# thuanz123/enhancing-transformers

Measured on AMD Instinct MI355X. Metric: images/sec ViT-VQGAN-base 256px stage-1 train; VQ argmin match-rate, higher is better.
Workload: dtype fp16; 1 GPU; imagenet_vitvq_base.yaml AE training step (1 fwd + 1 bwd + grad all-reduce + AdamW), loss = 1.0*L2 + 1.0*codebook (LPIPS/GAN weights 0), K=8192 x 32 l2-normalised codes, fp32 master weights, fp16 MFMA operands / fp32 accumulate, dynamic loss scale (now 65536; device-side inf/nan step skip + GradScaler update rule); per_gpu_batch=128, global_batch=128, image=256x256, parallelism=dp1, hip_graph_replay=False

## Files before the change

enhancing-transformers_amd/csrc/attention_kernels.h:

```cpp
#ifndef ATT_TAIL
#error "attention_kernels.h is included with ATT_TAIL (0 | 1) and ATT_K (the kernel names) defined"
#endif
#include "attention_tile_loop.h"

template <typename OT>
__device__ __forceinline__ void ATT_K(fwd, exact)(const uint16_t* __restrict__ qkv, int B, int N, int H, float scale_log2, uint16_t* __restrict__ out,
                                               float* __restrict__ lse, unsigned char (*smem)[2][ATT_TILE_BYTES], int blk, int head) {
  const int t = threadIdx.x, lane = t & 63, wave = t >> 6;
  const int l31 = lane & 31, hi = lane >> 5;
  const int b = head / H, h = head - b * H;
  const int q0 = blk * 128 + wave * 32;
  const int64_t RS = (int64_t)3 * H * ATT_D;
  const uint16_t* Qp = qkv + (int64_t)b * N * RS + h * ATT_D;
  const uint16_t* Kp = Qp + H * ATT_D;
  const uint16_t* Vp = Kp + H * ATT_D;

  const bool active = ATT_SEL(q0 + l31 < N, q0 < N);
  const int qrow = ATT_SEL(min(q0 + l31, N - 1), active ? q0 + l31 : l31);
  s16x8 qf[4];
#pragma unroll
  for (int ds = 0; ds < 4; ++ds) qf[ds] = *reinterpret_cast<const s16x8*>(Qp + (int64_t)qrow * RS + ds * 16 + hi * 8);

  f32x16 o[2];
#pragma unroll
  for (int db = 0; db < 2; ++db)
#pragma unroll
    for (int r = 0; r < 16; ++r) o[db][r] = 0.f;
  float m_run = -__builtin_inff(), l_part = 0.f;

  const int nt = N / 64;
  u32x4 rk[2], rv[2];
#if ATT_TAIL
  if (nt == 0) {
    att_gload_clamped(rk, Kp, RS, 0, N, t);
    att_gload_clamped(rv, Vp, RS, 0, N, t);
  } else
#endif
  {
  att_gload(rk, Kp, RS, 0, t);
  att_gload(rv, Vp, RS, 0, t);
  }
  att_sstore(rk, smem[0][0], t);
  att_sstore(rv, smem[0][1], t);
#pragma unroll
  for (int ds = 0; ds < 4; ++ds) att_pin(qf[ds]);
  ATT_LOOP_ENTRY();
  __syncthreads();
  ATT_TILES_BEGIN(kt, nt)
    const int st = kt & 1;
#if ATT_TAIL
    if constexpr (LAST) {
    } else if (kt + 1 == nt) {
      att_gload_clamped(rk, Kp, RS, (kt + 1) * 64, N, t);
      att_gload_clamped(rv, Vp, RS, (kt + 1) * 64, N, t);
    } else
#else
    if (kt + 1 < nt)
#endif
    {
      att_gload(rk, Kp, RS, (kt + 1) * 64, t);
      att_gload(rv, Vp, RS, (kt + 1) * 64, t);
    }
    const unsigned char* kt_ = smem[st][0];
    const unsigned char* vt_ = smem[st][1];
    f32x16 s[2];
#pragma unroll
    for (int kb = 0; kb < 2; ++kb) {
#pragma unroll
      for (int r = 0; r < 16; ++r) s[kb][r] = ATT_SEL(LAST ? att_key_bias(kb, r, hi, N & 63) : 0.f, 0.f);
#pragma unroll
      for (int ds = 0; ds < 4; ++ds) s[kb] = MFMA32(att_frag_row(kt_, kb * 32, ds, l31, hi), qf[ds], s[kb]);
    }
    float mx = max3(s[0][0], s[0][1], s[0][2]);
#pragma unroll
    for (int r = 3; r < 15; r += 2) mx = max3(mx, s[0][r], s[0][r + 1]);
    mx = max3(mx, s[0][15], s[1][0]);
#pragma unroll
    for (int r = 1; r < 15; r += 2) mx = max3(mx, s[1][r], s[1][r + 1]);
    mx = xhalf_max(__builtin_fmaxf(mx, s[1][15]));
    const float mt = mx * scale_log2;
    if (kt == 0 || __builtin_amdgcn_ballot_w64(mt - m_run > 8.0f) != 0) {
      const float m_new = fmaxf(m_run, mt);
      const float alpha = __builtin_amdgcn_exp2f(m_run - m_new);
      m_run = m_new;
      l_part *= alpha;
#pragma unroll
      for (int db = 0; db < 2; ++db)
#pragma unroll
        for (int r = 0; r < 16; ++r) o[db][r] *= alpha;
    }
    float p[2][16];
    float psum = 0.f;
#pragma unroll
    for (int kb = 0; kb < 2; ++kb)
#pragma unroll
      for (int r = 0; r < 16; ++r) {
        p[kb][r] = __builtin_amdgcn_exp2f(s[kb][r] * scale_log2 - m_run);
        psum += p[kb][r];
      }
    l_part += psum;
#pragma unroll
    for (int kb = 0; kb < 2; ++kb)
#pragma unroll
      for (int c2 = 0; c2 < 2; ++c2) {
        const s16x8 pb = pack8<OT>(&p[kb][c2 * 8]);
#pragma unroll
        for (int db = 0; db < 2; ++db) o[db] = MFMA32(att_frag_tr(vt_, kb * 32 + 16 * c2, db, lane), pb, o[db]);
      }
    ATT_UNLESS_LAST {
    if (ATT_SEL(true, kt + 1 < nt)) {
      att_sstore(rk, smem[st ^ 1][0], t);
      att_sstore(rv, smem[st ^ 1][1], t);
    }
    __syncthreads();
    }
  ATT_TILES_END(kt, nt)
  const float l = l_part + __shfl_xor(l_part, 32, 64);
  const float inv = 1.0f / l;
  if (!active) return;
  uint16_t* op = out + ((int64_t)b * N + q0 + l31) * (H * ATT_D) + h * ATT_D;
#pragma unroll
  for (int db = 0; db < 2; ++db)
#pragma unroll
    for (int g4 = 0; g4 < 4; ++g4) {
      const int d0 = db * 32 + 8 * g4 + 4 * hi;
      u32x2 w = {pack2<OT>(o[db][g4 * 4 + 0] * inv, o[db][g4 * 4 + 1] * inv), pack2<OT>(o[db][g4 * 4 + 2] * inv, o[db][g4 * 4 + 3] * inv)};
      *reinterpret_cast<u32x2*>(op + d0) = w;
    }
  if (hi == 0) lse[((int64_t)b * H + h) * N + q0 + l31] = (m_run + __builtin_amdgcn_logf(l)) * 0.6931471805599453f;
}

#define ATT_PF 1
__host__ __device__ constexpr bool att_run_start(int k, int P, bool WHOLE) { return k == 0 || (!WHOLE && (k % P == 0 || k % P == 8)); }
__host__ __device__ constexpr int att_run_end(int I, int NF, int P, bool WHOLE) {
  int e = I + 1;
  while (e < NF && !att_run_start(e, P, WHOLE)) ++e;
  return e;
}
__host__ __device__ constexpr int att_pending(int I, int NF, int P, bool WHOLE) {
  int n = 0;
  for (int k = I + 1; k <= I + ATT_PF && k < att_run_end(I, NF, P, WHOLE); ++k) n += (k % P < 8) ? 1 : 2;
  return n;
}
template <int I, int NF, int P, bool WHOLE, typename REQ>
__device__ __forceinline__ void att_stream_request(REQ& req) {
  constexpr int E = att_run_end(I, NF, P, WHOLE);
  if constexpr (att_run_start(I, P, WHOLE)) att_static_for<I, (I + ATT_PF < E ? I + ATT_PF : E)>(req);
  if constexpr (I + ATT_PF < E) req(std::integral_constant<int, I + ATT_PF>{});
}

template <typename OT>
__global__ __launch_bounds__(256, 2) void ATT_K(fwd, kernel)(const uint16_t* __restrict__ qkv, int B, int N, int H, float scale_log2,
                                                          uint16_t* __restrict__ out, float* __restrict__ lse) {
  __shared__ __attribute__((aligned(16))) unsigned char smem[2][2][ATT_TILE_BYTES];
  int blk, head;
  if (!att_block_coords((N + 127) / 128, B * H, blk, head)) return;
  ATT_K(fwd, exact)<OT>(qkv, B, N, H, scale_log2, out, lse, smem, blk, head);
}

__device__ __forceinline__ float dot2_ones(uint32_t pk, float acc) {
  return __builtin_amdgcn_fdot2_f32_bf16(__builtin_bit_cast(bf16x2_t, pk), __builtin_bit_cast(bf16x2_t, 0x3f803f80u), acc, false);
}
template <typename OT>
__global__ __launch_bounds__(256, 2) void ATT_K(fwd, pre_kernel)(const uint16_t* __restrict__ qkv, int B, int N, int H, uint16_t* __restrict__ out, float* __restrict__ lse) {
  __shared__ __attribute__((aligned(16))) unsigned char smem[2][2][ATT_TILE_BYTES];
  int blk, head;
  if (!att_block_coords((N + 127) / 128, B * H, blk, head)) return;
  const int t = threadIdx.x, lane = t & 63, wave = t >> 6;
  const int l31 = lane & 31, hi = lane >> 5;
  const int b = head / H, h = head - b * H;
  const int q0 = blk * 128 + wave * 32;
  const int64_t RS = (int64_t)3 * H * ATT_D;
  const uint16_t* Qp = qkv + (int64_t)b * N * RS + h * ATT_D;
  const uint16_t* Kp = Qp + H * ATT_D;
  const uint16_t* Vp = Kp + H * ATT_D;
  const bool active = ATT_SEL(q0 + l31 < N, q0 < N);
  const int qrow = ATT_SEL(min(q0 + l31, N - 1), active ? q0 + l31 : l31);
  s16x8 qf[4];
#pragma unroll
  for (int ds = 0; ds < 4; ++ds) qf[ds] = *reinterpret_cast<const s16x8*>(Qp + (int64_t)qrow * RS + ds * 16 + hi * 8);
  f32x16 o[2], negm;
#pragma unroll
  for (int r = 0; r < 16; ++r) { o[0][r] = 0.f; o[1][r] = 0.f; negm[r] = 0.f; }
  float m_ref = 0.f;
  f32x2 l2[2] = {{0.f, 0.f}, {0.f, 0.f}};

  const int nt = N / 64;
  const int wave_u = __builtin_amdgcn_readfirstlane(wave);
  const unsigned ko0 = att_dma_lane_off((int)RS, lane, 0), ko1 = att_dma_lane_off((int)RS, lane, 1);
#if ATT_TAIL
  if (nt == 0) {
    att_dma_tile_clamped(Kp, RS, 0, N, smem[0][0], wave_u, lane);
    att_dma_tile_clamped(Vp, RS, 0, N, smem[0][1], wave_u, lane);
  } else
#endif
  {
  att_dma_tile(Kp, RS, 0, smem[0][0], wave_u, ko0, ko1);
  att_dma_tile(Vp, RS, 0, smem[0][1], wave_u, ko0, ko1);
  }
  unsigned ra[4], ta[2][2];
  att_ring_addresses(ra, ta, &smem[0][0][0], lane);
#pragma unroll
  for (int ds = 0; ds < 4; ++ds) att_pin(qf[ds]);
  ATT_LOOP_ENTRY();
  __syncthreads();
  ATT_TILES_BEGIN(kt, nt)
    const int st = kt & 1;
#if ATT_TAIL
    if constexpr (LAST) {
    } else if (kt + 1 == nt) {
      att_dma_tile_clamped(Kp, RS, (kt + 1) * 64, N, smem[st ^ 1][0], wave_u, lane);
      att_dma_tile_clamped(Vp, RS, (kt + 1) * 64, N, smem[st ^ 1][1], wave_u, lane);
    } else
#else
    if (kt + 1 < nt)
#endif
    {
      att_dma_tile(Kp, RS, (kt + 1) * 64, smem[st ^ 1][0], wave_u, ko0, ko1);
      att_dma_tile(Vp, RS, (kt + 1) * 64, smem[st ^ 1][1], wave_u, ko0, ko1);
    }
    constexpr int NF = 16;
    u32x4 fr[ATT_PF + 1];
    att_u64 tl[ATT_PF + 1], th[ATT_PF + 1];
    auto req = [&](auto ic) {
      constexpr int I = decltype(ic)::value, B = I % (ATT_PF + 1);
      if constexpr (I < 8) att_req_row<(I >> 2) * 32 * 128>(fr[B], ra[I & 3]);
      else att_req_tr<ATT_TILE_BYTES + (((I - 8) >> 2) * 32 + 16 * (((I - 8) >> 1) & 1)) * 128>(tl[B], th[B], ta[I & 1][0], ta[I & 1][1]);
    };
    f32x16 s[2];
    att_static_for<0, 8>([&](auto ic) {
      constexpr int I = decltype(ic)::value, kb = I >> 2, ds = I & 3, B = I % (ATT_PF + 1);
      att_stream_request<I, NF, 16, false>(req);
#if ATT_TAIL
      if constexpr (LAST && ds == 0) {
#pragma unroll
        for (int r = 0; r < 16; ++r) s[kb][r] = negm[r] + att_key_bias(kb, r, hi, N & 63);
      }
#endif
      s[kb] = MFMA32(att_take_row<att_pending(I, NF, 16, false)>(fr[B]), qf[ds], ATT_SEL(ds == 0 && !LAST, ds == 0) ? negm : s[kb]);
    });
    float mq[4];
#pragma unroll
    for (int c = 0; c < 4; ++c) {
      const f32x16& sv = s[c >> 1];
      const int r0 = (c & 1) * 8;
      mq[c] = max3(sv[r0], sv[r0 + 1], sv[r0 + 2]);
      mq[c] = max3(mq[c], sv[r0 + 3], sv[r0 + 4]);
      mq[c] = max3(mq[c], sv[r0 + 5], sv[r0 + 6]);
    }
    float mx = max3(mq[0], mq[1], s[0][7]);
    mx = max3(mx, mq[2], s[0][15]);
    mx = max3(mx, mq[3], s[1][7]);
    mx = xhalf_max(__builtin_fmaxf(mx, s[1][15]));
    if (kt == 0 || __builtin_amdgcn_ballot_w64(mx > 8.0f) != 0) {
      const float delta = kt == 0 ? mx : __builtin_fmaxf(mx, 0.f);
      if (kt != 0) {
        const float alpha = __builtin_amdgcn_exp2f(-delta);
        l2[0] *= alpha; l2[1] *= alpha;
#pragma unroll
        for (int db = 0; db < 2; ++db)
#pragma unroll
          for (int r = 0; r < 16; ++r) o[db][r] *= alpha;
      }
      m_ref += delta;
#pragma unroll
      for (int r = 0; r < 16; ++r) { s[0][r] -= delta; s[1][r] -= delta; negm[r] = -m_ref; }
    }
    s16x8 pb;
    att_static_for<8, 16>([&](auto ic) {
      constexpr int I = decltype(ic)::value, kb = (I - 8) >> 2, c2 = ((I - 8) >> 1) & 1, db = I & 1, B = I % (ATT_PF + 1);
      att_stream_request<I, NF, 16, false>(req);
      if constexpr (db == 0) {
        float p8[8];
#pragma unroll
        for (int j = 0; j < 8; ++j) p8[j] = __builtin_amdgcn_exp2f(s[kb][c2 * 8 + j]);
        const u32x4 pk = {pack2<OT>(p8[0], p8[1]), pack2<OT>(p8[2], p8[3]), pack2<OT>(p8[4], p8[5]), pack2<OT>(p8[6], p8[7])};
#pragma unroll
        for (int j = 0; j < 4; ++j) l2[j & 1] += (f32x2){p8[2 * j], p8[2 * j + 1]};
        pb = __builtin_bit_cast(s16x8, pk);
      }
      o[db] = MFMA32(att_take_tr<att_pending(I, NF, 16, false)>(tl[B], th[B]), pb, o[db]);
    });
    ATT_UNLESS_LAST {
    att_ring_advance(ra, ta, st);
    ATT_FENCE();
    __builtin_amdgcn_s_waitcnt(0x0F70);
    __syncthreads();
    }
  ATT_TILES_END(kt, nt)
  const float l_part = (l2[0][0] + l2[1][0]) + (l2[0][1] + l2[1][1]);
  const float l = l_part + __shfl_xor(l_part, 32, 64);
  const float inv = 1.0f / l;
  if (!active) return;
  uint16_t* op = out + ((int64_t)b * N + q0 + l31) * (H * ATT_D) + h * ATT_D;
#pragma unroll
  for (int db = 0; db < 2; ++db)
#pragma unroll
    for (int g4 = 0; g4 < 4; ++g4) {
      const int d0 = db * 32 + 8 * g4 + 4 * hi;
      u32x2 w = {pack2<OT>(o[db][g4 * 4 + 0] * inv, o[db][g4 * 4 + 1] * inv), pack2<OT>(o[db][g4 * 4 + 2] * inv, o[db][g4 * 4 + 3] * inv)};
      *reinterpret_cast<u32x2*>(op + d0) = w;
    }
  if (hi == 0) lse[((int64_t)b * H + h) * N + q0 + l31] = (m_ref + __builtin_amdgcn_logf(l)) * 0.6931471805599453f;
}

template <int MODE, typename OT>
__global__ __launch_bounds__(256, 3) void ATT_K(bwd, dq_kernel)(const uint16_t* __restrict__ qkv, const uint16_t* __restrict__ o, const uint16_t* __restrict__ d_o,
                                                             const float* __restrict__ lse, float* __restrict__ delta, int B, int N,
                                                             int H, float scale, float scale_log2, uint16_t* __restrict__ dqkv) {
  __shared__ __attribute__((aligned(16))) unsigned char smem[2][2][ATT_TILE_BYTES];
  const int t = threadIdx.x, lane = t & 63, wave = t >> 6;
  const int l31 = lane & 31, hi = lane >> 5;
  int blk, head;
  if (!att_block_coords((N + 127) / 128, B * H, blk, head)) return;
  const int b = head / H, h = head - b * H;
  const int q0 = blk * 128 + wave * 32;
  const int64_t RS = (int64_t)3 * H * ATT_D;
  const uint16_t* Qp = qkv + (int64_t)b * N * RS + h * ATT_D;
  const uint16_t* Kp = Qp + H * ATT_D;
  const uint16_t* Vp = Kp + H * ATT_D;
  const uint16_t* dOp = d_o + (int64_t)b * N * (H * ATT_D) + h * ATT_D;

  const bool active = ATT_SEL(q0 + l31 < N, q0 < N);
  const int qrow = ATT_SEL(min(q0 + l31, N - 1), active ? q0 + l31 : l31);
  s16x8 qf[4], dof[4];
#pragma unroll
  for (int ds = 0; ds < 4; ++ds) {
    qf[ds] = *reinterpret_cast<const s16x8*>(Qp + (int64_t)qrow * RS + ds * 16 + hi * 8);
    dof[ds] = *reinterpret_cast<const s16x8*>(dOp + (int64_t)qrow * (H * ATT_D) + ds * 16 + hi * 8);
  }
  const float lse_q = lse[((int64_t)b * H + h) * N + qrow] * 1.4426950408889634f;
  float dpart = 0.f;
#pragma unroll
  for (int ds = 0; ds < 4; ++ds) {
    const s16x8 of = *reinterpret_cast<const s16x8*>(o + ((int64_t)b * N + qrow) * (H * ATT_D) + h * ATT_D + ds * 16 + hi * 8);
#pragma unroll
    for (int k = 0; k < 8; ++k) dpart += unpack1<OT>((uint16_t)of[k]) * unpack1<OT>((uint16_t)dof[ds][k]);
  }
  const float del_q = dpart + __shfl_xor(dpart, 32, 64);
  if (active && hi == 0) delta[((int64_t)b * H + h) * N + qrow] = del_q;
  f32x16 negd, negl;
#pragma unroll
  for (int r = 0; r < 16; ++r) { negd[r] = MODE >= 1 ? -del_q : 0.f; negl[r] = MODE == 2 ? -lse_q : 0.f; }

  f32x16 dq[2];
#pragma unroll
  for (int db = 0; db < 2; ++db)
#pragma unroll
    for (int r = 0; r < 16; ++r) dq[db][r] = 0.f;

  const int nt = N / 64;
  const int wave_u = __builtin_amdgcn_readfirstlane(wave);
  const unsigned ko0 = att_dma_lane_off((int)RS, lane, 0), ko1 = att_dma_lane_off((int)RS, lane, 1);
#if ATT_TAIL
  if (nt == 0) {
    att_dma_tile_clamped(Kp, RS, 0, N, smem[0][0], wave_u, lane);
    att_dma_tile_clamped(Vp, RS, 0, N, smem[0][1], wave_u, lane);
  } else
#endif
  {
  att_dma_tile(Kp, RS, 0, smem[0][0], wave_u, ko0, ko1);
  att_dma_tile(Vp, RS, 0, smem[0][1], wave_u, ko0, ko1);
  }
#pragma unroll
  for (int ds = 0; ds < 4; ++ds) { att_pin(qf[ds]); att_pin(dof[ds]); }
  ATT_LOOP_ENTRY();
  __syncthreads();
  unsigned ra[4], ta[2][2];
  att_ring_addresses(ra, ta, &smem[0][0][0], lane);
  ATT_TILES_BEGIN(kt, nt)
    const int st = kt & 1;
#if ATT_TAIL
    if constexpr (LAST) {
    } else if (kt + 1 == nt) {
      att_dma_tile_clamped(Kp, RS, (kt + 1) * 64, N, smem[st ^ 1][0], wave_u, lane);
      att_dma_tile_clamped(Vp, RS, (kt + 1) * 64, N, smem[st ^ 1][1], wave_u, lane);
    } else
#else
    if (kt + 1 < nt)
#endif
    {
      att_dma_tile(Kp, RS, (kt + 1) * 64, smem[st ^ 1][0], wave_u, ko0, ko1);
      att_dma_tile(Vp, RS, (kt + 1) * 64, smem[st ^ 1][1], wave_u, ko0, ko1);
    }
    constexpr int NF = 24;
    u32x4 fr[ATT_PF + 1];
    att_u64 tl[ATT_PF + 1], th[ATT_PF + 1];
    auto req = [&](auto ic) {
      constexpr int I = decltype(ic)::value, kb = I / 12, j = I % 12, B = I % (ATT_PF + 1);
      if constexpr (j < 8) att_req_row<(j & 1) * ATT_TILE_BYTES + kb * 32 * 128>(fr[B], ra[j >> 1]);
      else att_req_tr<(kb * 32 + 16 * ((j - 8) >> 1)) * 128>(tl[B], th[B], ta[j & 1][0], ta[j & 1][1]);
    };
    f32x16 s, dp;
    float dsv[16];
    s16x8 dsb;
    att_static_for<0, NF>([&](auto ic) {
      constexpr int I = decltype(ic)::value, j = I % 12, B = I % (ATT_PF + 1);
      att_stream_request<I, NF, 12, true>(req);
      constexpr int PEND = att_pending(I, NF, 12, true);
      if constexpr (j < 8) {
        constexpr int ds = j >> 1;
        const s16x8 f = att_take_row<PEND>(fr[B]);
#if ATT_TAIL
        if constexpr (LAST && j == 0) {
#pragma unroll
          for (int r = 0; r < 16; ++r) s[r] = negl[r] + att_key_bias(I / 12, r, hi, N & 63);
        }
#endif
        if constexpr ((j & 1) == 0) s = MFMA32(f, qf[ds], ATT_SEL(ds == 0 && !LAST, ds == 0) ? negl : s);
        else dp = MFMA32(f, dof[ds], ds == 0 ? negd : dp);
        if constexpr (j == 7) {
#pragma unroll
          for (int r = 0; r < 16; ++r) {
            const float pr = MODE == 2 ? __builtin_amdgcn_exp2f(s[r]) : __builtin_amdgcn_exp2f(s[r] * scale_log2 - lse_q);
            dsv[r] = MODE >= 1 ? pr * dp[r] : pr * (dp[r] - del_q);
          }
        }
      } else {
        constexpr int c2 = (j - 8) >> 1, db = j & 1;
        if constexpr (db == 0) dsb = pack8<OT>(&dsv[c2 * 8]);
        dq[db] = MFMA32(att_take_tr<PEND>(tl[B], th[B]), dsb, dq[db]);
      }
    });
    ATT_UNLESS_LAST {
    att_ring_advance(ra, ta, st);
    ATT_FENCE();
    __builtin_amdgcn_s_waitcnt(0x0F70);
    __syncthreads();
    }
  ATT_TILES_END(kt, nt)
  if (!active) return;
  uint16_t* op = dqkv + ((int64_t)b * N + q0 + l31) * RS + h * ATT_D;
#pragma unroll
  for (int db = 0; db < 2; ++db)
#pragma unroll
    for (int g4 = 0; g4 < 4; ++g4) {
      const int d0 = db * 32 + 8 * g4 + 4 * hi;
      u32x2 w = {pack2<OT>(dq[db][g4 * 4 + 0] * scale, dq[db][g4 * 4 + 1] * scale), pack2<OT>(dq[db][g4 * 4 + 2] * scale, dq[db][g4 * 4 + 3] * scale)};
      *reinterpret_cast<u32x2*>(op + d0) = w;
    }
}

template <bool CINIT, bool PRE, typename OT>
#ifndef ATT_DKV_OCC
#define ATT_DKV_OCC 2
#endif
__global__ __launch_bounds__(256, ATT_DKV_OCC) void ATT_K(bwd, dkv_kernel)(const uint16_t* __restrict__ qkv, const uint16_t* __restrict__ d_o,
                                                              const float* __restrict__ lse, const float* __restrict__ delta, int B, int N,
                                                              int H, float scale, float scale_log2, uint16_t* __restrict__ dqkv) {
  __shared__ __attribute__((aligned(16))) unsigned char smem[2][2][ATT_TILE_BYTES];
  __shared__ __attribute__((aligned(16))) float s_stat[2][2][64];
  const int t = threadIdx.x, lane = t & 63, wave = t >> 6;
  const int l31 = lane & 31, hi = lane >> 5;
  int blk, head;
  if (!att_block_coords((N + 127) / 128, B * H, blk, head)) return;
  const int b = head / H, h = head - b * H;
  const int key0 = blk * 128 + wave * 32;
  const int64_t RS = (int64_t)3 * H * ATT_D;
  const int64_t OS = (int64_t)H * ATT_D;
  const uint16_t* Qp = qkv + (int64_t)b * N * RS + h * ATT_D;
  const uint16_t* Kp = Qp + H * ATT_D;
  const uint16_t* Vp = Kp + H * ATT_D;
  const uint16_t* dOp = d_o + (int64_t)b * N * OS + h * ATT_D;
  const float* lsep = lse + ((int64_t)b * H + h) * N;
  const float* delp = delta + ((int64_t)b * H + h) * N;

  const bool active = ATT_SEL(key0 + l31 < N, key0 < N);
  const int krow = ATT_SEL(min(key0 + l31, N - 1), active ? key0 + l31 : l31);
  s16x8 kf[4], vf[4];
#pragma unroll
  for (int ds = 0; ds < 4; ++ds) {
    kf[ds] = *reinterpret_cast<const s16x8*>(Kp + (int64_t)krow * RS + ds * 16 + hi * 8);
    vf[ds] = *reinterpret_cast<const s16x8*>(Vp + (int64_t)krow * RS + ds * 16 + hi * 8);
  }
  f32x16 dk[2], dv[2];
#pragma unroll
  for (int db = 0; db < 2; ++db)
#pragma unroll
    for (int r = 0; r < 16; ++r) { dk[db][r] = 0.f; dv[db][r] = 0.f; }

  const int nt = ATT_SEL(N / 64 + 1, N / 64);
  const int wave_u = __builtin_amdgcn_readfirstlane(wave);
  const unsigned qo0 = att_dma_lane_off((int)RS, lane, 0), qo1 = att_dma_lane_off((int)RS, lane, 1);
  const unsigned do0 = att_dma_lane_off((int)OS, lane, 0), do1 = att_dma_lane_off((int)OS, lane, 1);
  float rstat = 0.f;
#if ATT_TAIL
  if (nt == 1) {
    att_dma_tile_clamped(Qp, RS, 0, N, smem[0][0], wave_u, lane);
    att_dma_tile_clamped(dOp, OS, 0, N, smem[0][1], wave_u, lane);
  } else
#endif
  {
  att_dma_tile(Qp, RS, 0, smem[0][0], wave_u, qo0, qo1);
  att_dma_tile(dOp, OS, 0, smem[0][1], wave_u, do0, do1);
  }
  unsigned ra[4], ta[2][2];
  att_ring_addresses(ra, ta, &smem[0][0][0], lane);
  const float* statp = ((t & 64) ? delp : lsep) + (t & 63);
  const float stat_mul = (t & 64) ? (CINIT ? -1.0f : 1.0f) : ((CINIT && PRE) ? -1.4426950408889634f : 1.4426950408889634f);
#if ATT_TAIL
  const float stat_masked = (t & 64) ? 0.f : ((CINIT && PRE) ? ATT_MASK_BIAS : -ATT_MASK_BIAS);
#endif
  rstat = statp[ATT_SEL(min(0, N - 1 - (t & 63)), 0)];
  if (t < 128) s_stat[0][t >> 6][t & 63] = ATT_SEL((t & 63) >= N ? stat_masked :, ) rstat * stat_mul;
#pragma unroll
  for (int ds = 0; ds < 4; ++ds) { att_pin(kf[ds]); att_pin(vf[ds]); }
  ATT_LOOP_ENTRY();
  __syncthreads();
  for (int qt = 0; qt < nt; ++qt) {
    const int st = qt & 1;
#if ATT_TAIL
    if (qt + 2 == nt) {
      att_dma_tile_clamped(Qp, RS, (qt + 1) * 64, N, smem[st ^ 1][0], wave_u, lane);
      att_dma_tile_clamped(dOp, OS, (qt + 1) * 64, N, smem[st ^ 1][1], wave_u, lane);
      rstat = statp[min((qt + 1) * 64, N - 1 - (t & 63))];
    }
#endif
    if (qt + 1 < ATT_SEL(nt - 1, nt)) {
      att_dma_tile(Qp, RS, (qt + 1) * 64, smem[st ^ 1][0], wave_u, qo0, qo1);
      att_dma_tile(dOp, OS, (qt + 1) * 64, smem[st ^ 1][1], wave_u, do0, do1);
      rstat = statp[(qt + 1) * 64];
    }
    constexpr int NF = 32;
    u32x4 fr[ATT_PF + 1];
    att_u64 tl[ATT_PF + 1], th[ATT_PF + 1];
    auto req = [&](auto ic) {
      constexpr int I = decltype(ic)::value, qb = I / 16, j = I % 16, B = I % (ATT_PF + 1);
      if constexpr (j < 8) att_req_row<(j & 1) * ATT_TILE_BYTES + qb * 32 * 128>(fr[B], ra[j >> 1]);
      else att_req_tr<((j & 1) ^ 1) * ATT_TILE_BYTES + (qb * 32 + 16 * ((j - 8) >> 2)) * 128>(tl[B], th[B], ta[(j >> 1) & 1][0], ta[(j >> 1) & 1][1]);
    };
    f32x16 s, dp, lrow, drow;
    float pv[16], dsv[16];
    s16x8 pa, dsa;
    att_static_for<0, NF>([&](auto ic) {
      constexpr int I = decltype(ic)::value, qb = I / 16, j = I % 16, B = I % (ATT_PF + 1);
      att_stream_request<I, NF, 16, true>(req);
      constexpr int PEND = att_pending(I, NF, 16, true);
      if constexpr (j == 0) {
#pragma unroll
        for (int g4 = 0; g4 < 4; ++g4) {
          const int row0 = qb * 32 + 8 * g4 + 4 * hi;
          const f32x4 l4 = *reinterpret_cast<const f32x4*>(&s_stat[st][0][row0]);
          const f32x4 d4 = *reinterpret_cast<const f32x4*>(&s_stat[st][1][row0]);
#pragma unroll
          for (int k = 0; k < 4; ++k) { lrow[g4 * 4 + k] = l4[k]; dp[g4 * 4 + k] = d4[k]; }
        }
        drow = dp;
        if (!(CINIT && PRE)) {
#pragma unroll
          for (int r = 0; r < 16; ++r) s[r] = 0.f;
        } else {
          s = lrow;
        }
        if (!CINIT) {
#pragma unroll
          for (int r = 0; r < 16; ++r) dp[r] = 0.f;
        }
      }
      if constexpr (j < 8) {
        constexpr int ds = j >> 1;
        const s16x8 f = att_take_row<PEND>(fr[B]);
        if constexpr ((j & 1) == 0) s = MFMA32(f, kf[ds], s);
        else dp = MFMA32(f, vf[ds], dp);
        if constexpr (j == 7) {
#pragma unroll
          for (int r = 0; r < 16; ++r) {
            pv[r] = (CINIT && PRE) ? __builtin_amdgcn_exp2f(s[r]) : __builtin_amdgcn_exp2f(s[r] * scale_log2 - lrow[r]);
            dsv[r] = CINIT ? pv[r] * dp[r] : pv[r] * (dp[r] - drow[r]);
          }
        }
      } else {
        constexpr int c2 = (j - 8) >> 2, db = (j >> 1) & 1;
        if constexpr (((j - 8) & 3) == 0) { pa = pack8<OT>(&pv[c2 * 8]); dsa = pack8<OT>(&dsv[c2 * 8]); }
        const s16x8 f = att_take_tr<PEND>(tl[B], th[B]);
        if constexpr ((j & 1) == 0) dv[db] = MFMA32(f, pa, dv[db]);
        else dk[db] = MFMA32(f, dsa, dk[db]);
      }
    });
    att_ring_advance(ra, ta, st);
    ATT_FENCE();
    __builtin_amdgcn_s_waitcnt(0x0F70);
    if (qt + 1 < nt && t < 128) s_stat[st ^ 1][t >> 6][t & 63] = ATT_SEL((qt + 1) * 64 + (t & 63) >= N ? stat_masked :, ) rstat * stat_mul;
    __syncthreads();
  }
  if (!active) return;
  uint16_t* dkp = dqkv + ((int64_t)b * N + key0 + l31) * RS + H * ATT_D + h * ATT_D;
  uint16_t* dvp = dkp + H * ATT_D;
#pragma unroll
  for (int db = 0; db < 2; ++db)
#pragma unroll
    for (int g4 = 0; g4 < 4; ++g4) {
      const int d0 = db * 32 + 8 * g4 + 4 * hi;
      const u32x2 wk = {pack2<OT>(dk[db][g4 * 4 + 0] * scale, dk[db][g4 * 4 + 1] * scale), pack2<OT>(dk[db][g4 * 4 + 2] * scale, dk[db][g4 * 4 + 3] * scale)};
      const u32x2 wv = {pack2<OT>(dv[db][g4 * 4 + 0], dv[db][g4 * 4 + 1]), pack2<OT>(dv[db][g4 * 4 + 2], dv[db][g4 * 4 + 3])};
      *reinterpret_cast<u32x2*>(dkp + d0) = wk;
      *reinterpret_cast<u32x2*>(dvp + d0) = wv;
    }
}
```

Baseline: 621.9 images/s.

## Interleave softmax exp and dS packing with MFMA issue in attention backward kernels

Reorders the dq and dkv backward inner loops so that the S and dP MFMAs for the key/query sub-block are issued first. The exp2 and dS computation is then split into two-row chunks placed between later MFMA issues, with fences around them, so that VALU transcendental work overlaps with matrix-core work instead of running as a serialized block after each sub-block. The LDS row/stat loads for the second sub-block are moved to mid-loop. The tail-path dq epilogue recomputes lane coordinates from an opaque copy of the thread id, probably to reduce live registers. This raises register pressure (two s/dp accumulators per loop) and could hurt occupancy.

Result: no change. 626.4 images/s, median of 6 (+0.7%).

```diff
diff --git a/enhancing-transformers_amd/csrc/attention_kernels.h b/enhancing-transformers_amd/csrc/attention_kernels.h
--- a/enhancing-transformers_amd/csrc/attention_kernels.h
+++ b/enhancing-transformers_amd/csrc/attention_kernels.h
@@ -137,9 +137,9 @@
   while (e < NF && !att_run_start(e, P, WHOLE)) ++e;
   return e;
 }
-__host__ __device__ constexpr int att_pending(int I, int NF, int P, bool WHOLE) {
+__host__ __device__ constexpr int att_pending(int I, int NF, int P, bool WHOLE, int R = 8) {
   int n = 0;
-  for (int k = I + 1; k <= I + ATT_PF && k < att_run_end(I, NF, P, WHOLE); ++k) n += (k % P < 8) ? 1 : 2;
+  for (int k = I + 1; k <= I + ATT_PF && k < att_run_end(I, NF, P, WHOLE); ++k) n += (k % P < R) ? 1 : 2;
   return n;
 }
 template <int I, int NF, int P, bool WHOLE, typename REQ>
@@ -387,39 +387,50 @@
     u32x4 fr[ATT_PF + 1];
     att_u64 tl[ATT_PF + 1], th[ATT_PF + 1];
     auto req = [&](auto ic) {
-      constexpr int I = decltype(ic)::value, kb = I / 12, j = I % 12, B = I % (ATT_PF + 1);
-      if constexpr (j < 8) att_req_row<(j & 1) * ATT_TILE_BYTES + kb * 32 * 128>(fr[B], ra[j >> 1]);
-      else att_req_tr<(kb * 32 + 16 * ((j - 8) >> 1)) * 128>(tl[B], th[B], ta[j & 1][0], ta[j & 1][1]);
-    };
-    f32x16 s, dp;
-    float dsv[16];
-    s16x8 dsb;
+      constexpr int I = decltype(ic)::value, B = I % (ATT_PF + 1);
+      if constexpr (I < 16) att_req_row<((I >> 2) & 1) * ATT_TILE_BYTES + (I >> 3) * 32 * 128>(fr[B], ra[I & 3]);
+      else att_req_tr<(((I - 16) >> 2) * 32 + 16 * (((I - 16) >> 1) & 1)) * 128>(tl[B], th[B], ta[I & 1][0], ta[I & 1][1]);
+    };
+    f32x16 s[2], dp[2];
+    float pe[2][16];
+    u32x4 dsw[2][2];
+    auto expo = [&](auto uc) {
+      constexpr int U = decltype(uc)::value, kb = U >> 3, r0 = (U & 7) * 2;
+#pragma unroll
+      for (int r = r0; r < r0 + 2; ++r) pe[kb][r] = MODE == 2 ? __builtin_amdgcn_exp2f(s[kb][r]) : __builtin_amdgcn_exp2f(s[kb][r] * scale_log2 - lse_q);
+    };
+    auto fin = [&](auto uc) {
+      constexpr int U = decltype(uc)::value, kb = U >> 3, p = U & 7, r0 = p * 2;
+      float d[2];
+#pragma unroll
+      for (int k = 0; k < 2; ++k) d[k] = MODE >= 1 ? pe[kb][r0 + k] * dp[kb][r0 + k] : pe[kb][r0 + k] * (dp[kb][r0 + k] - del_q);
+      dsw[kb][p >> 2][p & 3] = pack2<OT>(d[0], d[1]);
+    };
     att_static_for<0, NF>([&](auto ic) {
-      constexpr int I = decltype(ic)::value, j = I % 12, B = I % (ATT_PF + 1);
-      att_stream_request<I, NF, 12, true>(req);
-      constexpr int PEND = att_pending(I, NF, 12, true);
-      if constexpr (j < 8) {
-        constexpr int ds = j >> 1;
+      constexpr int I = decltype(ic)::value, B = I % (ATT_PF + 1);
+      att_stream_request<I, NF, 24, true>(req);
+      constexpr int PEND = att_pending(I, NF, 24, true, 16);
+      if constexpr (I < 16) {
+        constexpr int kb = I >> 3, ds = I & 3;
         const s16x8 f = att_take_row<PEND>(fr[B]);
 #if ATT_TAIL
-        if constexpr (LAST && j == 0) {
-#pragma unroll
-          for (int r = 0; r < 16; ++r) s[r] = negl[r] + att_key_bias(I / 12, r, hi, N & 63);
+        if constexpr (LAST && (I & 7) == 0) {
+#pragma unroll
+          for (int r = 0; r < 16; ++r) s[kb][r] = negl[r] + att_key_bias(kb, r, hi, N & 63);
         }
 #endif
-        if constexpr ((j & 1) == 0) s = MFMA32(f, qf[ds], ATT_SEL(ds == 0 && !LAST, ds == 0) ? negl : s);
-        else dp = MFMA32(f, dof[ds], ds == 0 ? negd : dp);
-        if constexpr (j == 7) {
-#pragma unroll
-          for (int r = 0; r < 16; ++r) {
-            const float pr = MODE == 2 ? __builtin_amdgcn_exp2f(s[r]) : __builtin_amdgcn_exp2f(s[r] * scale_log2 - lse_q);
-            dsv[r] = MODE >= 1 ? pr * dp[r] : pr * (dp[r] - del_q);
-          }
-        }
+        if constexpr ((I & 4) == 0) s[kb] = MFMA32(f, qf[ds], ATT_SEL(ds == 0 && !LAST, ds == 0) ? negl : s[kb]);
+        else dp[kb] = MFMA32(f, dof[ds], ds == 0 ? negd : dp[kb]);
       } else {
-        constexpr int c2 = (j - 8) >> 1, db = j & 1;
-        if constexpr (db == 0) dsb = pack8<OT>(&dsv[c2 * 8]);
-        dq[db] = MFMA32(att_take_tr<PEND>(tl[B], th[B]), dsb, dq[db]);
+        constexpr int kb = (I - 16) >> 2, c2 = ((I - 16) >> 1) & 1, db = I & 1;
+        dq[db] = MFMA32(att_take_tr<PEND>(tl[B], th[B]), __builtin_bit_cast(s16x8, dsw[kb][c2]), dq[db]);
+      }
+      if constexpr (I >= 4 && I <= 19) {
+        constexpr int U = 8 * ((I - 4) >> 3) + 2 * (I & 3);
+        ATT_FENCE();
+        if constexpr ((I & 4) != 0) { expo(std::integral_constant<int, U>{}); expo(std::integral_constant<int, U + 1>{}); }
+        else { fin(std::integral_constant<int, U>{}); fin(std::integral_constant<int, U + 1>{}); }
+        ATT_FENCE();
       }
     });
     ATT_UNLESS_LAST {
@@ -429,13 +440,21 @@
     __syncthreads();
     }
   ATT_TILES_END(kt, nt)
+#if ATT_TAIL
+  int te = t;
+  asm volatile("" : "+v"(te));
+  const int l31e = te & 31, hie = (te >> 5) & 1, q0e = blk * 128 + (te >> 6) * 32;
+  if (q0e + l31e >= N) return;
+  uint16_t* op = dqkv + ((int64_t)b * N + q0e + l31e) * RS + h * ATT_D;
+#else
   if (!active) return;
   uint16_t* op = dqkv + ((int64_t)b * N + q0 + l31) * RS + h * ATT_D;
+#endif
 #pragma unroll
   for (int db = 0; db < 2; ++db)
 #pragma unroll
     for (int g4 = 0; g4 < 4; ++g4) {
-      const int d0 = db * 32 + 8 * g4 + 4 * hi;
+      const int d0 = db * 32 + 8 * g4 + 4 * ATT_SEL(hie, hi);
       u32x2 w = {pack2<OT>(dq[db][g4 * 4 + 0] * scale, dq[db][g4 * 4 + 1] * scale), pack2<OT>(dq[db][g4 * 4 + 2] * scale, dq[db][g4 * 4 + 3] * scale)};
       *reinterpret_cast<u32x2*>(op + d0) = w;
     }
@@ -525,56 +544,88 @@
     u32x4 fr[ATT_PF + 1];
     att_u64 tl[ATT_PF + 1], th[ATT_PF + 1];
     auto req = [&](auto ic) {
-      constexpr int I = decltype(ic)::value, qb = I / 16, j = I % 16, B = I % (ATT_PF + 1);
-      if constexpr (j < 8) att_req_row<(j & 1) * ATT_TILE_BYTES + qb * 32 * 128>(fr[B], ra[j >> 1]);
-      else att_req_tr<((j & 1) ^ 1) * ATT_TILE_BYTES + (qb * 32 + 16 * ((j - 8) >> 2)) * 128>(tl[B], th[B], ta[(j >> 1) & 1][0], ta[(j >> 1) & 1][1]);
-    };
-    f32x16 s, dp, lrow, drow;
-    float pv[16], dsv[16];
-    s16x8 pa, dsa;
+      constexpr int I = decltype(ic)::value, B = I % (ATT_PF + 1);
+      constexpr int qb = I >> 4, o = I & 15;
+      if constexpr (o < 8) att_req_row<(o >> 2) * ATT_TILE_BYTES + qb * 32 * 128>(fr[B], ra[o & 3]);
+      else att_req_tr<(((o >> 2) & 1) ^ 1) * ATT_TILE_BYTES + (qb * 32 + 16 * ((o >> 1) & 1)) * 128>(tl[B], th[B], ta[o & 1][0], ta[o & 1][1]);
+    };
+    f32x16 s[2], dp[2], lrow[2], drow[2];
+    float pe[2][16];
+    u32x4 pw[2][2], dsw[2][2];
+    auto stat = [&](auto qbc, auto wc) {
+      constexpr int qb = decltype(qbc)::value, W = decltype(wc)::value;
+      f32x16 v;
+#pragma unroll
+      for (int g4 = 0; g4 < 4; ++g4) {
+        const f32x4 x4 = *reinterpret_cast<const f32x4*>(&s_stat[st][W][qb * 32 + 8 * g4 + 4 * hi]);
+#pragma unroll
+        for (int k = 0; k < 4; ++k) v[g4 * 4 + k] = x4[k];
+      }
+      if constexpr (W == 0) {
+        lrow[qb] = v;
+        if (!(CINIT && PRE)) {
+#pragma unroll
+          for (int r = 0; r < 16; ++r) s[qb][r] = 0.f;
+        } else {
+          s[qb] = v;
+        }
+      } else {
+        drow[qb] = v;
+        if (!CINIT) {
+#pragma unroll
+          for (int r = 0; r < 16; ++r) dp[qb][r] = 0.f;
+        } else {
+          dp[qb] = v;
+        }
+      }
+    };
+    auto expo = [&](auto uc) {
+      constexpr int U = decltype(uc)::value, qb = U >> 3, p = U & 7, r0 = p * 2;
+#pragma unroll
+      for (int r = r0; r < r0 + 2; ++r)
+        pe[qb][r] = (CINIT && PRE) ? __builtin_amdgcn_exp2f(s[qb][r]) : __builtin_amdgcn_exp2f(s[qb][r] * scale_log2 - lrow[qb][r]);
+    };
+    auto ppack = [&](auto uc) {
+      constexpr int U = decltype(uc)::value, qb = U >> 3, p = U & 7, r0 = p * 2;
+      pw[qb][p >> 2][p & 3] = pack2<OT>(pe[qb][r0], pe[qb][r0 + 1]);
+    };
+    auto fin = [&](auto uc) {
+      constexpr int U = decltype(uc)::value, qb = U >> 3, p = U & 7, r0 = p * 2;
+      float d[2];
+#pragma unroll
+      for (int k = 0; k < 2; ++k) d[k] = CINIT ? pe[qb][r0 + k] * dp[qb][r0 + k] : pe[qb][r0 + k] * (dp[qb][r0 + k] - drow[qb][r0 + k]);
+      dsw[qb][p >> 2][p & 3] = pack2<OT>(d[0], d[1]);
+    };
     att_static_for<0, NF>([&](auto ic) {
-      constexpr int I = decltype(ic)::value, qb = I / 16, j = I % 16, B = I % (ATT_PF + 1);
+      constexpr int I = decltype(ic)::value, qb = I >> 4, o = I & 15, B = I % (ATT_PF + 1);
       att_stream_request<I, NF, 16, true>(req);
       constexpr int PEND = att_pending(I, NF, 16, true);
-      if constexpr (j == 0) {
-#pragma unroll
-        for (int g4 = 0; g4 < 4; ++g4) {
-          const int row0 = qb * 32 + 8 * g4 + 4 * hi;
-          const f32x4 l4 = *reinterpret_cast<const f32x4*>(&s_stat[st][0][row0]);
-          const f32x4 d4 = *reinterpret_cast<const f32x4*>(&s_stat[st][1][row0]);
-#pragma unroll
-          for (int k = 0; k < 4; ++k) { lrow[g4 * 4 + k] = l4[k]; dp[g4 * 4 + k] = d4[k]; }
-        }
-        drow = dp;
-        if (!(CINIT && PRE)) {
-#pragma unroll
-          for (int r = 0; r < 16; ++r) s[r] = 0.f;
-        } else {
-          s = lrow;
-        }
-        if (!CINIT) {
-#pragma unroll
-          for (int r = 0; r < 16; ++r) dp[r] = 0.f;
-        }
-      }
-      if constexpr (j < 8) {
-        constexpr int ds = j >> 1;
+      if constexpr (I == 0) { stat(std::integral_constant<int, 0>{}, std::integral_constant<int, 0>{}); stat(std::integral_constant<int, 0>{}, std::integral_constant<int, 1>{}); }
+      if constexpr (o < 8) {
+        constexpr int ds = o & 3;
         const s16x8 f = att_take_row<PEND>(fr[B]);
-        if constexpr ((j & 1) == 0) s = MFMA32(f, kf[ds], s);
-        else dp = MFMA32(f, vf[ds], dp);
-        if constexpr (j == 7) {
-#pragma unroll
-          for (int r = 0; r < 16; ++r) {
-            pv[r] = (CINIT && PRE) ? __builtin_amdgcn_exp2f(s[r]) : __builtin_amdgcn_exp2f(s[r] * scale_log2 - lrow[r]);
-            dsv[r] = CINIT ? pv[r] * dp[r] : pv[r] * (dp[r] - drow[r]);
-          }
-        }
+        if constexpr (o < 4) s[qb] = MFMA32(f, kf[ds], s[qb]);
+        else dp[qb] = MFMA32(f, vf[ds], dp[qb]);
       } else {
-        constexpr int c2 = (j - 8) >> 2, db = (j >> 1) & 1;
-        if constexpr (((j - 8) & 3) == 0) { pa = pack8<OT>(&pv[c2 * 8]); dsa = pack8<OT>(&dsv[c2 * 8]); }
+        constexpr int c2 = (o >> 1) & 1, db = o & 1;
         const s16x8 f = att_take_tr<PEND>(tl[B], th[B]);
-        if constexpr ((j & 1) == 0) dv[db] = MFMA32(f, pa, dv[db]);
-        else dk[db] = MFMA32(f, dsa, dk[db]);
+        if constexpr (o < 12) dv[db] = MFMA32(f, __builtin_bit_cast(s16x8, pw[qb][c2]), dv[db]);
+        else dk[db] = MFMA32(f, __builtin_bit_cast(s16x8, dsw[qb][c2]), dk[db]);
+      }
+      if constexpr (o >= 4 && o <= 11) {
+        constexpr int U = 8 * qb + 2 * (o & 3);
+        ATT_FENCE();
+        if constexpr (o < 8) { expo(std::integral_constant<int, U>{}); expo(std::integral_constant<int, U + 1>{}); }
+        else { fin(std::integral_constant<int, U>{}); fin(std::integral_constant<int, U + 1>{}); }
+        if constexpr (o == 4 || o == 5) { ppack(std::integral_constant<int, U>{}); ppack(std::integral_constant<int, U + 1>{}); }
+        if constexpr (o == 8 || o == 9) { ppack(std::integral_constant<int, U + 4>{}); ppack(std::integral_constant<int, U + 5>{}); }
+        ATT_FENCE();
+      }
+      if constexpr (I == 13) {
+        ATT_FENCE();
+        stat(std::integral_constant<int, 1>{}, std::integral_constant<int, 0>{});
+        stat(std::integral_constant<int, 1>{}, std::integral_constant<int, 1>{});
+        ATT_FENCE();
       }
     });
     att_ring_advance(ra, ta, st);
```
